# zhangganlin/GlobalSfMpy

Measured on AMD Instinct MI355X. Metric: edge_residuals_per_sec, higher is better.
Workload: dtype f64

## Files before the change

### globalsfmpy_amd/csrc/colsort_kernels.hpp

```cpp
#pragma once
#include "kernels.hpp"

namespace gsfm {

#define GSFM_COL_RB 512
#define GSFM_COL_SUB GSFM_COL_RB
#define GSFM_COL_SLOT_BITS 9
static_assert(GSFM_COL_RB == (1 << GSFM_COL_SLOT_BITS), "row blocks of 512 rows");
#ifndef GSFM_COL_EPL
#define GSFM_COL_EPL 1
#endif
#define GSFM_COL_PAD 0xffffffffu

struct ColWg { uint32_t first_sub, n_sub, row0, part; };
struct ColLayoutDev {
  const ColWg* wg;
  const uint2* meta;
  const uint32_t* kcol;
  const uint16_t* kcnt;
  uint32_t cbits, cmax;
  uint32_t n_wg, nch;
  const uint16_t* k16;
  const uint32_t* kbase;
  const uint32_t* kdel;
};
#define GSFM_K16_CNT_ESC 7u
#define GSFM_K16_DEL_ESC 15u
__host__ __device__ constexpr uint32_t col_pack(uint32_t slot, uint32_t rowcount, uint32_t rowl) { return slot | (rowcount << GSFM_COL_SLOT_BITS) | (rowl << (2 * GSFM_COL_SLOT_BITS + 1)); }
__host__ __device__ __forceinline__ uint32_t col_slot(uint32_t y) { return y & ((1u << GSFM_COL_SLOT_BITS) - 1u); }
__host__ __device__ __forceinline__ uint32_t col_rowcount(uint32_t y) { return (y >> GSFM_COL_SLOT_BITS) & ((2u << GSFM_COL_SLOT_BITS) - 1u); }
__host__ __device__ __forceinline__ uint32_t col_rowl(uint32_t y) { return y >> (2 * GSFM_COL_SLOT_BITS + 1); }
__device__ __forceinline__ uint32_t wave_incl_scan(uint32_t x) {
  int v = (int)x;
  v += __builtin_amdgcn_update_dpp(0, v, 0x111, 0xf, 0xf, false);
  v += __builtin_amdgcn_update_dpp(0, v, 0x112, 0xf, 0xf, false);
  v += __builtin_amdgcn_update_dpp(0, v, 0x114, 0xf, 0xf, false);
  v += __builtin_amdgcn_update_dpp(0, v, 0x118, 0xf, 0xf, false);
  v += __builtin_amdgcn_update_dpp(0, v, 0x142, 0xa, 0xf, false);
  v += __builtin_amdgcn_update_dpp(0, v, 0x143, 0xc, 0xf, false);
  return (uint32_t)v;
}

__device__ __forceinline__ uint2 col_load_meta(const uint2* p) {
  uint2 v;
  v.x = __builtin_nontemporal_load(&p->x); v.y = __builtin_nontemporal_load(&p->y);
  return v;
}

struct ColMatvecArgs {
  ColLayoutDev L;
  const double2 *b0, *b1, *b2;
  const double* u;
  double* part;
  const int* done;
};
template <bool K16, typename Stop>
__device__ __forceinline__ void mv_col_body(const ColMatvecArgs& a, Stop stop_after_request) {
  constexpr int RB = GSFM_COL_RB, EPL = GSFM_COL_EPL;
  __shared__ double slots[2][EPL][3][RB];
  __shared__ uint32_t wtot[2][EPL][RB / 64];
  const ColWg w = a.L.wg[blockIdx.x];
  const uint32_t r = threadIdx.x, wave = r >> 6;
  double y0 = 0.0, y1 = 0.0, y2 = 0.0;
  uint32_t m[EPL], pos[EPL], cbase[EPL]; double2 A[EPL], B[EPL], C[EPL];
  const uint32_t cmask = (1u << a.L.cbits) - 1u, cshift = a.L.cbits + GSFM_COL_SLOT_BITS, cmax = a.L.cmax;
  auto request = [&](uint32_t s) {
#pragma unroll
    for (int k = 0; k < EPL; ++k) {
      const uint32_t sc = w.first_sub + min(s + (uint32_t)k, w.n_sub - 1);
      const size_t e = (size_t)sc * RB + r;
      pos[k] = (uint32_t)e;
      if constexpr (K16) { m[k] = __builtin_nontemporal_load(a.L.k16 + e); cbase[k] = a.L.kbase[(size_t)sc * (RB / 64) + __builtin_amdgcn_readfirstlane(wave)]; }
      else { m[k] = __builtin_nontemporal_load(a.L.kcol + e); cbase[k] = 0u; }
      A[k] = nt_load2(a.b0 + e); B[k] = nt_load2(a.b1 + e); C[k] = nt_load2(a.b2 + e);
    }
  };
  if (w.n_sub) request(0);
  if (stop_after_request()) return;
  int buf = 0;
  for (uint32_t s = 0; s < w.n_sub; s += EPL, buf ^= 1) {
    uint32_t cnt[EPL], inc[EPL];
#pragma unroll
    for (int k = 0; k < EPL; ++k) {
      uint32_t cam, pm, c;
      if constexpr (K16) {
        uint32_t dl = m[k] >> 12;
        if (dl == GSFM_K16_DEL_ESC) dl = a.L.kdel[pos[k]];
        cam = cbase[k] + wave_incl_scan(dl);
        pm = m[k] & ((1u << GSFM_COL_SLOT_BITS) - 1u);
        c = (m[k] >> GSFM_COL_SLOT_BITS) & 7u;
        if (c == GSFM_K16_CNT_ESC) c = a.L.kcnt[pos[k]];
      } else {
        cam = (m[k] & cmask) == cmask ? 0u : (m[k] & cmask); pm = (m[k] >> a.L.cbits) & ((1u << GSFM_COL_SLOT_BITS) - 1u);
        c = m[k] >> cshift;
        if (c == cmax) c = a.L.kcnt[pos[k]];
      }
      const double* um = a.u + 3 * (size_t)cam;
      const double u0 = um[0], u1 = um[1], u2 = um[2];
      slots[buf][k][0][pm] = A[k].x * u0 + A[k].y * u1 + B[k].x * u2;
      slots[buf][k][1][pm] = A[k].y * u0 + B[k].y * u1 + C[k].x * u2;
      slots[buf][k][2][pm] = B[k].x * u0 + C[k].x * u1 + C[k].y * u2;
      cnt[k] = s + (uint32_t)k < w.n_sub ? c : 0u;
      inc[k] = wave_incl_scan(cnt[k]);
      if ((r & 63u) == 63u) wtot[buf][k][wave] = inc[k];
    }
    if (s + EPL < w.n_sub) request(s + EPL);
    __syncthreads();
#pragma unroll
    for (int k = 0; k < EPL; ++k) {
      uint32_t s1 = inc[k];
      for (uint32_t v = 0; v < wave; ++v) s1 += wtot[buf][k][v];
      for (uint32_t t = s1 - cnt[k]; t < s1; ++t) { y0 += slots[buf][k][0][t]; y1 += slots[buf][k][1][t]; y2 += slots[buf][k][2][t]; }
    }
  }
  const size_t o = (size_t)w.part * RB + r, plane = (size_t)a.L.n_wg * RB;
  a.part[o] = y0; a.part[plane + o] = y1; a.part[2 * plane + o] = y2;
}
#define GSFM_K3C_THREADS GSFM_COL_RB
template <bool K16>
__global__ void __launch_bounds__(GSFM_K3C_THREADS) k_mv_col(ColMatvecArgs a) {
  if (a.done && *a.done) return;
  mv_col_body<K16>(a, [] { return false; });
}
struct ColMatvecCgArgs { ColMatvecArgs mv; Cg2Args cg; };
template <bool K16>
__global__ void __launch_bounds__(GSFM_K3C_THREADS) k_mv_col_cg(ColMatvecCgArgs aa) {
  __shared__ double lds[4];
  const Cg2Args& c = aa.cg;
  mv_col_body<K16>(aa.mv, [&]() -> bool {
    const int done = c.sc->done, iters = c.sc->iters;
    const double gamma0 = c.sc->gamma0, tol = c.sc->tol;
    const bool estop = cg_energy_stop(c.sc->einc, c.sc->esum, c.sc->etol2, iters);
    double gpart = 0.0;
    if (threadIdx.x < GSFM_BLOCK) for (int k = threadIdx.x; k < c.nb_cam; k += GSFM_BLOCK) gpart += c.part_g[(size_t)c.par * c.nb_cam + k];
    gpart = wave_sum(gpart);
    if ((threadIdx.x & 63u) == 0 && threadIdx.x < GSFM_BLOCK) lds[threadIdx.x >> 6] = gpart;
    __syncthreads();
    double gamma = 0.0;
#pragma unroll
    for (int k = 0; k < GSFM_BLOCK / 64; ++k) gamma += lds[k];
    if (done) return true;
    bool conv;
    if (c.first) {
      const double rz_abs = c.sc->rz_abs;
      conv = !(gamma > rz_abs);
      if (blockIdx.x == 0 && threadIdx.x == 0) { c.sc->gamma0 = gamma; c.sc->tol = cg_tol_with_floor(tol, rz_abs, gamma); if (conv) { c.sc->done = 1; c.sc->last_rel = 0.0; } }
    } else {
      const double rel = sqrt(gamma / gamma0);
      conv = !(rel > tol) || iters >= c.max_iters || estop;
      if (blockIdx.x == 0 && threadIdx.x == 0) { c.sc->last_rel = rel; if (conv) c.sc->done = 1; }
    }
    return conv;
  });
}
struct ColFinishArgs {
  uint32_t n_rows, row_base, nch, n_wg;
  const double* part; const double* Mblk; const double* p; const double2* q; double* y; const int* done;
  double* dot_part;
};
__global__ void __launch_bounds__(GSFM_BLOCK) k_mv_col_finish(ColFinishArgs a) {
  if (a.done && *a.done) return;
  __shared__ double lds[8];
  const uint32_t row = blockIdx.x * GSFM_BLOCK + threadIdx.x;
  double pAp = 0.0;
  if (row < a.n_rows) {
  const uint32_t blk = row / GSFM_COL_RB, r = row % GSFM_COL_RB;
  const size_t plane = (size_t)a.n_wg * GSFM_COL_RB;
  double t0 = 0.0, t1 = 0.0, t2 = 0.0;
  constexpr uint32_t FB = 8;
  for (uint32_t c0 = 0; c0 < a.nch; c0 += FB) {
    double v0[FB], v1[FB], v2[FB];
#pragma unroll
    for (uint32_t j = 0; j < FB; ++j) {
      const size_t o = ((size_t)blk * a.nch + min(c0 + j, a.nch - 1)) * GSFM_COL_RB + r;
      v0[j] = a.part[o]; v1[j] = a.part[plane + o]; v2[j] = a.part[2 * plane + o];
    }
#pragma unroll
    for (uint32_t j = 0; j < FB; ++j) if (c0 + j < a.nch) { t0 += v0[j]; t1 += v1[j]; t2 += v2[j]; }
  }
  const size_t k = a.row_base + row;
  double R[9], mp[3];
  qmat(load_q(a.q, (uint32_t)k), R);
  sym3_mulvec(a.Mblk + 6 * k, a.p + 3 * k, mp);
  const double y0 = mp[0] - (R[0] * t0 + R[1] * t1 + R[2] * t2), y1 = mp[1] - (R[3] * t0 + R[4] * t1 + R[5] * t2), y2 = mp[2] - (R[6] * t0 + R[7] * t1 + R[8] * t2);
  a.y[3 * k] = y0; a.y[3 * k + 1] = y1; a.y[3 * k + 2] = y2;
  pAp = a.p[3 * k] * y0 + a.p[3 * k + 1] * y1 + a.p[3 * k + 2] * y2;
  }
  if (a.dot_part) {
    const double t = block_sum_bcast(pAp, lds);
    if (threadIdx.x == 0) a.dot_part[blockIdx.x] = t;
  }
}

struct ColRowSArgs {
  ColLayoutDev L;
  uint32_t row_base, n_rows;
  const uint32_t* eid;
  const double2 *qr0, *qr1, *w0, *w1, *w2;
  const double* ws;
  const double2* q;
  double* s_out;
};
template <int F, int WM>
__global__ void __launch_bounds__(GSFM_BLOCK) k_col_s(ColRowSArgs a) {
  constexpr int R = ResDim<F>::R;
  const ColWg w = a.L.wg[blockIdx.x];
  for (uint32_t d = w.first_sub * GSFM_COL_SUB + threadIdx.x; d < (w.first_sub + w.n_sub) * GSFM_COL_SUB; d += GSFM_BLOCK) {
    const uint2 mt = col_load_meta(a.L.meta + d);
    if (mt.x == GSFM_COL_PAD) continue;
    const Quat qk = load_q(a.q, a.row_base + w.row0 + col_rowl(mt.y)), qm = load_q(a.q, mt.x & 0x7fffffffu);
    double2 r0, r1;
    qrel_load<WM>(a.qr0, a.qr1, d, r0, r1);
    const Quat qr = qrel_quat<WM>(r0, r1);
    const EdgeW W = load_w<WM>(a.w0, a.w1, a.w2, a.ws, d);
    double r[R];
    if (mt.x >> 31) edge_residual<F, WM>(qm, qk, qr, W, r);
    else edge_residual<F, WM>(qk, qm, qr, W, r);
    double s = 0.0;
#pragma unroll
    for (int c = 0; c < R; ++c) s += r[c] * r[c];
// ... 229 lines not shown
```

### globalsfmpy_amd/csrc/host_common.hpp

```cpp
#pragma once

#include <dlfcn.h>
#include <hip/hip_runtime.h>

#include <algorithm>
#include <exception>
#include <functional>
#include <stdexcept>
#include <chrono>
#include <cmath>
#include <cstdio>
#include <cstdlib>
#include <cstring>
#include <limits>
#include <sched.h>
#include <string>
#include <thread>
#include <atomic>
#include <vector>

#include "../../include/gsfm_rot.h"
#include "kernels.hpp"
#include "cov_kernels.hpp"
#include "dense_kernels.hpp"
// ... 171 lines not shown
  void destroy() { if (ok) for (int k = 0; k < 2 * NPAIR; ++k) (void)hipEventDestroy(ev[k]); ok = false; }
  int begin(int category) {
    if (!ok || mute || mute_all) return -1;
    if (used == NPAIR) { (void)hipStreamSynchronize(stream); resolve(); }
    const int k = used++;
    cat[k] = category;
    (void)hipEventRecord(ev[2 * k], stream);
    return k;
  }
  void end(int k) { if (k >= 0) (void)hipEventRecord(ev[2 * k + 1], stream); }
  void resolve() {
    for (int k = 0; k < used; ++k) { float ms = 0; if (hipEventElapsedTime(&ms, ev[2 * k], ev[2 * k + 1]) == hipSuccess) acc[cat[k]] += ms; }
    used = 0;
  }
};


}

struct gsfm_rot_problem {
  uint32_t n_cams = 0;
  uint64_t n_edges_in = 0;
  int error_type = 0, functor = F_AA, wmode = W_NONE, param_dim = 3, res_dim = 3;
  bool sharded = false;
  gsfm_rot_shard shard{};
  uint32_t own_begin = 0, own_end = 0, n_rows = 0, n_pad = 0;
  int device = 0;
  hipStream_t stream = nullptr;
  bool own_stream = false;
  struct PcgGraph {
    struct Key {
      int max_iters = 0, stall = 0, chunk = 0; uint32_t coarse = 0; bool lap = false;
      const void* planes = nullptr;
      bool operator==(const Key& k) const { return max_iters == k.max_iters && stall == k.stall && chunk == k.chunk && coarse == k.coarse && lap == k.lap && planes == k.planes; }
    };
    hipGraphExec_t exec = nullptr;
    Key key;
    int collectives = 0;
    bool unusable = false;
    void reset() { if (exec) (void)hipGraphExecDestroy(exec); exec = nullptr; }
  } pcg_graph, pcg2_graph;
  PcgGraph pcg_graph_b, pcg2_graph_b;
  void reset_pcg_graphs() { pcg_graph.reset(); pcg2_graph.reset(); pcg_graph_b.reset(); pcg2_graph_b.reset(); }

  bool q3 = false;
  EdgePlanes cost;
  double cost_n_global = 0.0;
  DevBuf<uint2> cost_idx;
  DevBuf<CostTile> cost_tiles;
  const double2* q_lin = nullptr;
  bool lap = false, lap_capable = false, lin_is_lap = false;
  DevBuf<double> u_rot;
  std::vector<uint32_t> perm;
  std::vector<double> h_cam;
  DevBuf<uint32_t> d_perm;
  int cost_direct = 0;
  EdgePlanes dir;
  DevBuf<uint32_t> row_ptr, col;
  uint32_t G = 16;
  DevBuf<double2> h0, h1, h2, h3;
  DevBuf<double> h4;
  DevBuf<double2> h0_b, h1_b, h2_b;
  DevBuf<double> gD_b;
  int lin_set = 0;
  std::vector<uint32_t> h_cost_eid;

  DevBuf<double> x, x_trial, aa_io, active, scale, gD, Mblk, Minv, Lam, Tinv, b, D6;
// ... 44 lines not shown
  uint64_t loss_epoch = 0;
  hipGraphExec_t dense_graph = nullptr;
  bool dense_graph_lap = false;
  const void* dense_graph_planes = nullptr;
  int nb_mv = 1, mv_reps = 1;
  bool packed = false;
  bool pcg_local = false;
  DevBuf<double> b_own;
  bool component_rest = true;
  uint32_t n_components = 1;
  DevBuf<double> part_a, part_b, part_cost, part_cam, part_gauge, scal;
  DevBuf<CgScalars> cgsc;
  int nb_cam = 1, nb_cost = 1;

  DevLoss h_loss{};
  DevBuf<DevLoss> d_loss;
  DevBuf<double> tables[3];
  gsfm_loss_callback cb = nullptr;
  void* cb_user = nullptr;
  DevBuf<double> rho_ext, s_ext, w_orig;
  std::vector<double> h_s, h_rho;

  struct ColSort {
    bool active = false;
    uint32_t nch = 0, n_wg = 0;
    size_t n_pos = 0;
    DevBuf<ColWg> wg;
    DevBuf<uint2> meta;
    DevBuf<uint32_t> kcol;
    DevBuf<uint16_t> kcnt;
    uint32_t cbits = 0, cmax = 0;
    DevBuf<double> part;
    DevBuf<double> cost_part;
    bool k16_active = false;
    DevBuf<uint16_t> k16;
    DevBuf<uint32_t> kbase, kdel;
    ColLayoutDev dev() const { return ColLayoutDev{wg.p, meta.p, kcol.p, kcnt.p, cbits, cmax, n_wg, nch, k16_active ? k16.p : nullptr, kbase.p, kdel.p}; }
  } cs;

  SigmaDev sigma{};
  bool sigma_pending_cost = false, sigma_pending_lin = false;
  DevBuf<double> sigma_table, sigma_sum;

  bool have_lin = false;
  double* rec_host = nullptr;
  double* rec_dev = nullptr;
  double* mail_host = nullptr;
  double* mail_dev = nullptr;
  DevBuf<double> mail_count;
  double mail_expected = 0.0;
  int mail_state = 0;
  bool loss_staircase = false;
  bool loss_cuts_off = false;
  bool fast_lin_ok = true;
  int graph_launches = 0;
  int n_collectives = 0, n_pcg_collectives = 0, n_pcg_launched = 0;
  std::vector<double> trace;
  EventTimer timer;
};
```

### globalsfmpy_amd/csrc/kernels.hpp

```cpp
#pragma once
#include <hip/hip_runtime.h>
#include <stdint.h>
#include "loss_dev.hpp"
#include "so3_dev.hpp"

namespace gsfm {

enum { F_AA = 0, F_QCOS = 1, F_QNORM = 2, F_RFNORM = 3 };
enum { W_NONE = 0, W_SCALAR = 1, W_MATRIX = 2, W_MATRIX3 = 3  };

template <int F> struct ResDim { static constexpr int R = (F == F_QNORM) ? 4 : (F == F_RFNORM) ? 9 : 3; };

#define GSFM_BLOCK 256
#define GSFM_MAX_PARTIALS 1024
#define GSFM_CAMBLOCK 2048
#ifndef GSFM_TILE_THREADS
#define GSFM_TILE_THREADS 1024
#endif
#ifndef GSFM_K2_ATTR
#define GSFM_K2_ATTR __attribute__((amdgpu_waves_per_eu(3)))
#endif
#ifndef GSFM_GATHER_LOAD
#define GSFM_GATHER_LOAD(p) (*(p))
#endif
// ... 1228 lines not shown
      qt = aa_to_quat(x0, x1, x2);
    } else {
      const size_t k4 = 4 * (size_t)k;
      const Quat q{a.x[k4], a.x[k4 + 1], a.x[k4 + 2], a.x[k4 + 3]};
      const double nd = sqrt(d[0] * d[0] + d[1] * d[1] + d[2] * d[2]);
      qt = q;
      if (nd > 0.0) {
        double sn, cs;
        sincos(nd, &sn, &cs);
        const double kk = sn / nd;
        qt = qmul(Quat{kk * d[0], kk * d[1], kk * d[2], cs}, q);
      }
      a.x_trial[k4] = qt.x; a.x_trial[k4 + 1] = qt.y; a.x_trial[k4 + 2] = qt.z; a.x_trial[k4 + 3] = qt.w;
      const double f0 = q.x - qt.x, f1 = q.y - qt.y, f2 = q.z - qt.z, f3 = q.w - qt.w;
      v[3] = f0 * f0 + f1 * f1 + f2 * f2 + f3 * f3;
      v[4] = act * (qt.x * qt.x + qt.y * qt.y + qt.z * qt.z + qt.w * qt.w);
    }
    a.q_trial[2 * (size_t)k] = make_double2(qt.x, qt.y);
    a.q_trial[2 * (size_t)k + 1] = make_double2(qt.z, qt.w);
  }
#pragma unroll
  for (int c = 0; c < 6; ++c) {
    const double t = block_sum_bcast(v[c], lds);
    if (threadIdx.x == 0) a.partials[(size_t)c * gridDim.x + blockIdx.x] = t;
  }
}
__global__ void __launch_bounds__(GSFM_BLOCK) k_sum_partials_multi(const double* __restrict__ partials, int n, int m, double* out) {
  __shared__ double lds[8];
  for (int c = 0; c < m; ++c) {
    const double t = sum_partials_bcast(partials + (size_t)c * n, n, lds);
    if (threadIdx.x == 0) out[c] = t;
  }
}
__global__ void __launch_bounds__(GSFM_BLOCK) k_cam_norm(const double* __restrict__ x, const double* __restrict__ active,
                                                         uint32_t n, int param_dim, double* partials) {
  __shared__ double lds[8];
  double v = 0.0;
  const uint32_t k = blockIdx.x * GSFM_BLOCK + threadIdx.x;
  if (k < n && active[k] != 0.0) {
    for (int c = 0; c < param_dim; ++c) { const double t = x[(size_t)param_dim * k + c]; v += t * t; }
  }
  const double t = block_sum_bcast(v, lds);
  if (threadIdx.x == 0) partials[blockIdx.x] = t;
}

__global__ void __launch_bounds__(GSFM_BLOCK) k_cam_export(const double* __restrict__ x, const double* __restrict__ gD,
                                                           uint32_t n, int param_dim, double* grad, double* blocks, double* D6) {
  const uint32_t k = blockIdx.x * GSFM_BLOCK + threadIdx.x;
  if (k >= n) return;
  double T[9], Ti[9];
  cam_tangent_maps(x, k, param_dim, T, Ti);
  const double* gd = gD + 9 * (size_t)k;
  const double D[9] = {gd[3], gd[4], gd[5], gd[4], gd[6], gd[7], gd[5], gd[7], gd[8]};
  double DT[9], TDT[9];
  mat3_mul(D, T, DT);
  mat3_tmul(T, DT, TDT);
  for (int c = 0; c < 3; ++c) grad[3 * (size_t)k + c] = T[c] * gd[0] + T[3 + c] * gd[1] + T[6 + c] * gd[2];
  for (int c = 0; c < 9; ++c) blocks[9 * (size_t)k + c] = TDT[c];
  for (int c = 0; c < 6; ++c) D6[6 * (size_t)k + c] = gd[3 + c];
}
__global__ void __launch_bounds__(GSFM_BLOCK) k_cam_apply_T(const double* __restrict__ x, uint32_t n, int param_dim, int transpose,
                                                            const double* __restrict__ in, double* __restrict__ out) {
  const uint32_t k = blockIdx.x * GSFM_BLOCK + threadIdx.x;
  if (k >= n) return;
  double T[9], Ti[9];
  cam_tangent_maps(x, k, param_dim, T, Ti);
// ... 848 lines not shown
```

### globalsfmpy_amd/csrc/problem_create.hpp

```cpp
#pragma once
#include "host_common.hpp"

namespace {

template <typename AdjVec>
bool reorder_for_locality(uint32_t n_cams, uint64_t n_edges, const uint32_t* ei, const uint32_t* ej, const std::vector<uint32_t>& ptr,
                          const AdjVec& adj , std::vector<uint32_t>* perm) {
  perm->clear();
  const char* env = getenv("GSFM_REORDER");
  const int mode = env ? atoi(env) : -1;
  if (mode == 0 || (mode < 0 && n_cams < 2048)) return false;
  double before = 0.0;
  for (uint64_t e = 0; e < n_edges; ++e) before += std::fabs((double)ei[e] - (double)ej[e]);
  before /= (double)n_edges;
  if (mode < 0 && before < 256.0) return false;
  std::vector<uint32_t> stamp(n_cams, 0xffffffffu);
  if (mode < 0) {
    const uint32_t cap = n_cams / 8;
    int flooded = 0;
    for (uint32_t s = 0; s < 32; ++s) {
      const uint32_t c0 = (uint32_t)(((uint64_t)s * n_cams) / 32);
      uint32_t seen = 0;
      for (uint32_t d = ptr[c0]; d < ptr[c0 + 1] && seen < cap; ++d) {
        const uint32_t c1 = adj[d] & 0x7fffffffu;
// ... 142 lines not shown
          const size_t o = base + (e - lo);
          const uint32_t p = (uint32_t)(e - lo), rc = cnt[p + 1] - cnt[p];
          if (e < hi) {
            const uint32_t rl = (uint32_t)(ent[e].first & 0xffff), d = ent[e].second;
            h_col[o] = col[d]; h_eid[o] = deid[d]; h_meta[o] = make_uint2(col[d], col_pack(fill[rl]++, rc, rl));
          } else { h_col[o] = GSFM_COL_PAD; h_eid[o] = 0; h_meta[o] = make_uint2(GSFM_COL_PAD, col_pack(pad_slot++, rc, 0)); }
          h_kcol[o] = (h_meta[o].x == GSFM_COL_PAD ? kpad : (h_meta[o].x & 0x7fffffffu)) | (col_slot(h_meta[o].y) << cbits) | (std::min(rc, cmax) << (cbits + GSFM_COL_SLOT_BITS));
          h_kcnt[o] = (uint16_t)rc;
        }
        if (k16_mode != 0) {
          uint32_t prev = 0, esc = 0;
          for (uint32_t p = 0; p < SUB; ++p) {
            const size_t o = base + p;
            const uint32_t cam = h_meta[o].x == GSFM_COL_PAD ? prev : (h_meta[o].x & 0x7fffffffu);
            uint32_t step = 0;
            if ((p & 63u) == 0) h_kbase[(sub_off[b] + s) * (SUB / 64) + (p >> 6)] = cam; else step = cam - prev;
            prev = cam;
            const uint32_t rc = h_kcnt[o];
            h_kdel[o] = step;
            esc += (step >= GSFM_K16_DEL_ESC) + (rc >= GSFM_K16_CNT_ESC);
            h_k16[o] = (uint16_t)(col_slot(h_meta[o].y) | (std::min(rc, GSFM_K16_CNT_ESC) << GSFM_COL_SLOT_BITS) | (std::min(step, GSFM_K16_DEL_ESC) << 12));
          }
          k16_escapes.fetch_add(esc, std::memory_order_relaxed);
        }
      }
    }
  });
  C.n_wg = (uint32_t)h_wg.size(); C.n_pos = n_pos; C.cbits = cbits; C.cmax = cmax;
  if (k16_mode != 0 && (k16_mode > 0 || (double)k16_escapes.load() <= 0.01 * (double)n_pos)) {
    if (C.k16.upload(h_k16) == hipSuccess && C.kbase.upload(h_kbase) == hipSuccess && C.kdel.upload(h_kdel) == hipSuccess) C.k16_active = true;
    else { (void)hipGetLastError(); C.k16.release(); C.kbase.release(); C.kdel.release(); }
  }
  if (C.wg.upload(h_wg) != hipSuccess || C.meta.upload(h_meta) != hipSuccess || (!C.k16_active && C.kcol.upload(h_kcol) != hipSuccess) || C.kcnt.upload(h_kcnt) != hipSuccess ||
      C.part.alloc((size_t)9 * C.n_wg * RB) != hipSuccess) {
    (void)hipGetLastError();
    C = gsfm_rot_problem::ColSort();
    return 0;
  }
  if (getenv("GSFM_CREATE_TIMING")) fprintf(stderr, "gsfm create: column-sorted layout, %zu positions, 2-byte record %s (%llu escapes)\n", n_pos, C.k16_active ? "on" : "off", (unsigned long long)k16_escapes.load());
  col.swap(h_col); deid.swap(h_eid);
  C.active = true;
  return 0;
}

void run_whiten(gsfm_rot_problem* P, EdgePlanes& pl, const double* d_cov6, const double* d_inl) {
  if (P->wmode == W_NONE || pl.n == 0) return;
  WhitenArgs a{};
  a.cov6 = d_cov6; a.inl = d_inl; a.eid = pl.eid.p; a.n = pl.n; a.error_type = P->error_type;
  a.w0 = pl.w0.p; a.w1 = pl.w1.p; a.w2 = pl.w2.p; a.ws = pl.ws.p;
  hipLaunchKernelGGL(k_whiten, dim3(grid_for(pl.n)), dim3(GSFM_BLOCK), 0, P->stream, a);
}


static gsfm_status problem_create_impl(uint32_t n_cams, uint64_t n_edges, const uint32_t* edge_i_in, const uint32_t* edge_j_in,
                                       const double* rel_aa, int32_t error_type, const double* cov6, const double* inlier_weight,
                                       const gsfm_rot_shard* shard, gsfm_rot_problem** out, gsfm_rot_problem** live) {
  if (!out) return (gsfm_status)fail(GSFM_ERR_INVALID_ARG, "out is NULL");
  *out = nullptr;
  const bool multi_rank = shard && (shard->world_size > 1 || (shard->world_size == 1 && getenv("GSFM_FORCE_SHARD")));
  if (multi_rank && (!shard->all_gather || !shard->all_reduce_sum)) return (gsfm_status)fail(GSFM_ERR_INVALID_ARG, "bad shard descriptor: missing collective callbacks");
  if (const char* why = no_device_reason("the rotation solver")) return (gsfm_status)fail(GSFM_ERR_NO_DEVICE, why);

  gsfm_rot_problem* P = new gsfm_rot_problem;
  *live = P;
  bool agreed = false;
  DevBuf<double> agree_buf;
  double coarse_votes_against = 0.0;
// ... 403 lines not shown
```

### globalsfmpy_amd/csrc/solver_launch.hpp

```cpp
#pragma once
#include "host_common.hpp"

namespace {

int loss_mode(const gsfm_rot_problem* P) {
  if (P->cb) return LM_SIMPLE;
  const DevLoss& L = P->h_loss;
  if (L.n == 0) return LM_SIMPLE;
  if (L.n == 1) {
    const int k = L.nodes[0].kind;
    if (k == GSFM_LOSS_MAGSAC) return (L.nodes[0].nu == 3 && !L.nodes[0].inverse) ? LM_MAGSAC : LM_PROGRAM;
    if (k == GSFM_LOSS_TRIVIAL || k == GSFM_LOSS_HUBER || k == GSFM_LOSS_SOFT_L1 || k == GSFM_LOSS_TUKEY || k == GSFM_LOSS_GEMAN_MCCLURE) return LM_SIMPLE;
  }
  return LM_PROGRAM;
}
template <typename ArgsT, template <int, int, int> class Launcher>
int dispatch(const gsfm_rot_problem* P, const ArgsT& args, int grid) {
  const int f = P->functor, w = (P->wmode == W_MATRIX && P->q3) ? W_MATRIX3 : P->wmode, l = loss_mode(P);
#define GSFM_CASE3(F, W, L) if (f == F && w == W && l == L) { Launcher<F, W, L>::go(args, grid, P->stream); return 0; }
#define GSFM_CASE(F, W) GSFM_CASE3(F, W, LM_PROGRAM) GSFM_CASE3(F, W, LM_SIMPLE) GSFM_CASE3(F, W, LM_MAGSAC)
  GSFM_CASE(F_AA, W_NONE) GSFM_CASE(F_AA, W_SCALAR) GSFM_CASE(F_AA, W_MATRIX) GSFM_CASE(F_AA, W_MATRIX3)
  GSFM_CASE(F_QCOS, W_NONE) GSFM_CASE(F_QNORM, W_NONE) GSFM_CASE(F_RFNORM, W_NONE)
#undef GSFM_CASE
#undef GSFM_CASE3
// ... 248 lines not shown
      CostArgs a = cost_args(P, q);
      a.s_out = P->s_ext.p; a.s_only = 1; a.sigma = P->sigma; a.sigma.on = 1;
      if (dispatch<CostArgs, CostLauncher>(P, a, P->nb_cost)) return fail(GSFM_ERR_UNSUPPORTED, "no kernel for this error type");
      hipLaunchKernelGGL(k_sum_partials, dim3(1), dim3(GSFM_BLOCK), 0, P->stream, P->part_cost.p + P->nb_cost, P->nb_cost, P->sigma_sum.p);
      gsfm_loss_callback keep = P->cb;
      P->cb = nullptr;
      P->sigma_pending_lin = true;
      const int st = launch_lin(P, q);
      P->cb = keep;
      if (st) return st;
    }
    if (int st = refresh_external_rho(P, q)) return st;
  }
  CostArgs a = cost_args(P, q);
  a.rho_ext = P->cb ? P->rho_ext.p : nullptr;
  a.srho_out = out.srho; a.rho12_out = out.rho12; a.rho1_out = out.rho1; a.r_out = out.r; a.s_only = 0;
  if (sig && !P->cb) { a.sigma = P->sigma; a.sigma.on = 1; }
  const int tk = P->timer.begin(T_SWEEP);
  if (dispatch<CostArgs, CostLauncher>(P, a, P->nb_cost)) return fail(GSFM_ERR_UNSUPPORTED, "no kernel for this error type");
  P->timer.end(tk);
  if (reduce) hipLaunchKernelGGL(k_sum_partials, dim3(1), dim3(GSFM_BLOCK), 0, P->stream, P->part_cost.p, P->nb_cost, P->scal.p + slot);
  if (sig && !P->cb) hipLaunchKernelGGL(k_sum_partials, dim3(1), dim3(GSFM_BLOCK), 0, P->stream, P->part_cost.p + P->nb_cost, P->nb_cost, P->sigma_sum.p);
  return all_reduce(P, P->scal.p + slot, 1);
}

bool trial_lin_supported(const gsfm_rot_problem* P) {
  const char* e = getenv("GSFM_TRIAL_LIN");
  if (e && *e && atoi(e) == 0) return false;
  if (!P->h0_b.p || !P->cs.cost_part.p || P->sharded || P->cb || !P->cs.active || !P->lap || P->sigma_pending_cost || P->sigma_pending_lin || !k2_fast_path(P)) return false;
  const int w = (P->wmode == W_MATRIX && P->q3) ? W_MATRIX3 : P->wmode;
  return col_lin_cost_kernel(P->functor, w, loss_mode(P));
}

int launch_lin(gsfm_rot_problem* P, const double2* q, const double* go, bool fused, bool spare) {
  if (fused && !trial_lin_supported(P)) return fail(GSFM_ERR_UNSUPPORTED, "fused trial evaluation without its preconditions");
  if (P->cb) { if (int st = refresh_external_rho(P, q)) return st; }
  LinArgs a{};
  a.n_rows = P->n_rows; a.row_base = P->own_begin; a.G = P->G; a.row_ptr = P->row_ptr.p; a.col = P->col.p; a.eid = P->dir.eid.p;
  a.qr0 = P->dir.qr0.p; a.qr1 = P->dir.qr1.p; a.w0 = P->dir.w0.p; a.w1 = P->dir.w1.p; a.w2 = P->dir.w2.p; a.ws = P->dir.ws.p; a.ws_rw = P->dir.ws.p;
  a.q = q; a.loss = P->d_loss.p; a.rho_ext = P->cb ? P->rho_ext.p : nullptr; a.fast_ok = k2_fast_path(P) ? 1 : 0; a.go = go;
  if (P->sigma_pending_lin) { a.sigma = P->sigma; a.sigma.on = 1; P->sigma_pending_lin = false; }
  if (!P->lap && !P->h3.p && (P->h3.alloc(P->dir.n) != hipSuccess || P->h4.alloc(P->dir.n) != hipSuccess)) return fail(GSFM_ERR_HIP, "allocating the general normal-equation blocks failed");
  a.h0 = P->h0.p; a.h1 = P->h1.p; a.h2 = P->h2.p; a.h3 = P->h3.p; a.h4 = P->h4.p; a.gD = P->gD.p; a.lap = P->lap;
  if (spare) { a.h0 = P->h0_b.p; a.h1 = P->h1_b.p; a.h2 = P->h2_b.p; a.gD = P->gD_b.p; }
  else { P->lin_is_lap = P->lap; P->q_lin = q; }
  const int tk = P->timer.begin(T_LIN);
  if (P->cs.active) {
    ColLinArgs ca{};
    ca.lin = a; ca.L = P->cs.dev(); ca.part = P->cs.part.p; ca.cost_part = fused ? P->cs.cost_part.p : nullptr;
    if (dispatch<ColLinArgs, ColLinLauncher>(P, ca, (int)P->cs.n_wg)) return fail(GSFM_ERR_UNSUPPORTED, "no kernel for this error type");
    const bool body = col_lin_body_frame(P->functor, loss_mode(P) != LM_PROGRAM && !a.rho_ext && a.fast_ok);
    hipLaunchKernelGGL(k_lin_col_finish, dim3(grid_for(P->n_rows)), dim3(GSFM_BLOCK), 0, P->stream, P->n_rows, P->own_begin, P->cs.nch, P->cs.n_wg, (const double*)P->cs.part.p, a.gD,
                       body ? q : (const double2*)nullptr);
  } else if (dispatch<LinArgs, LinLauncher>(P, a, grid_for((size_t)P->n_rows * P->G))) return fail(GSFM_ERR_UNSUPPORTED, "no kernel for this error type");
  P->timer.end(tk);
  if (spare) return 0;
  P->have_lin = true;
  return all_gather(P, P->gD.p, (size_t)P->shard.slice_width * 9);
}

void accept_trial_lin(gsfm_rot_problem* P) {
  std::swap(P->h0.p, P->h0_b.p); std::swap(P->h1.p, P->h1_b.p); std::swap(P->h2.p, P->h2_b.p); std::swap(P->gD.p, P->gD_b.p);
  P->lin_set ^= 1;
  P->lin_is_lap = P->lap; P->q_lin = P->q.p;
  P->have_lin = true;
}

void launch_prep(gsfm_rot_problem* P, const gsfm_rot_options& o, double radius, bool init_scale, const double* radius_dev = nullptr, bool reduce = true) {
  PrepArgs a{};
  a.radius_dev = radius_dev;
  a.n = P->n_cams; a.param_dim = P->param_dim; a.x = P->x.p; a.gD = P->gD.p; a.scale = P->scale.p;
  a.init_scale = init_scale; a.jacobi_scaling = o.jacobi_scaling; a.radius = radius; a.min_diag = o.min_lm_diagonal; a.max_diag = o.max_lm_diagonal;
  a.Mblk = P->Mblk.p; a.Minv = P->Minv.p; a.Lam = P->Lam.p; a.Tinv = P->Tinv.p; a.b = P->b.p; a.gmax_partials = P->part_cam.p;
  hipLaunchKernelGGL(k_cam_prep, dim3(P->nb_cam), dim3(GSFM_BLOCK), 0, P->stream, a);
  if (reduce) {
    hipLaunchKernelGGL(k_max_partials, dim3(1), dim3(GSFM_BLOCK), 0, P->stream, P->part_cam.p, P->nb_cam, P->scal.p + SC_GMAX);
    double* part = P->part_cam.p + (size_t)5 * P->nb_cam;
    hipLaunchKernelGGL(k_cam_bound, dim3(P->nb_cam), dim3(GSFM_BLOCK), 0, P->stream, (const double*)P->Minv.p, (const double*)P->Tinv.p, (const double*)P->active.p, P->n_cams, part);
    hipLaunchKernelGGL(k_max_partials, dim3(1), dim3(GSFM_BLOCK), 0, P->stream, (const double*)part, P->nb_cam, P->scal.p + SC_ZBOUND);
  }
}

int launch_matvec(gsfm_rot_problem* P, const double* Mblk, const double* p, double* y, const int* done, double* dot_part = nullptr, bool* dot_done = nullptr) {
  if (dot_done) *dot_done = false;
  MatvecArgs a{};
  a.n_rows = P->n_rows; a.row_base = P->own_begin; a.G = P->G; a.row_ptr = P->row_ptr.p; a.col = P->col.p;
  a.h0 = P->h0.p; a.h1 = P->h1.p; a.h2 = P->h2.p; a.h3 = P->h3.p; a.h4 = P->h4.p; a.Mblk = Mblk; a.p = p; a.y = y; a.done = done;
  a.q = P->q_lin; a.u = P->u_rot.p;
  if (P->cs.active) {
    auto& c = P->cs;
    ColMatvecArgs m{};
    m.L = c.dev(); m.b0 = P->h0.p; m.b1 = P->h1.p; m.b2 = P->h2.p; m.u = P->u_rot.p; m.part = c.part.p; m.done = done;
    if (c.k16_active) hipLaunchKernelGGL(k_mv_col<true>, dim3(c.n_wg), dim3(GSFM_K3C_THREADS), 0, P->stream, m);
    else hipLaunchKernelGGL(k_mv_col<false>, dim3(c.n_wg), dim3(GSFM_K3C_THREADS), 0, P->stream, m);
    ColFinishArgs f{};
    f.n_rows = P->n_rows; f.row_base = P->own_begin; f.nch = c.nch; f.n_wg = c.n_wg; f.part = c.part.p; f.Mblk = Mblk; f.p = p; f.q = P->q_lin; f.y = y; f.done = done;
    if (dot_part && !P->sharded) { f.dot_part = dot_part; *dot_done = true; }
    hipLaunchKernelGGL(k_mv_col_finish, dim3(grid_for(P->n_rows)), dim3(GSFM_BLOCK), 0, P->stream, f);
    return P->pcg_local ? 0 : all_gather(P, y, (size_t)P->shard.slice_width * 3);
  }
  if (P->lin_is_lap) hipLaunchKernelGGL(k_matvec<true>, dim3(grid_for((size_t)P->n_rows * P->G)), dim3(GSFM_BLOCK), 0, P->stream, a);
  else hipLaunchKernelGGL(k_matvec<false>, dim3(grid_for((size_t)P->n_rows * P->G)), dim3(GSFM_BLOCK), 0, P->stream, a);
  return P->pcg_local ? 0 : all_gather(P, y, (size_t)P->shard.slice_width * 3);
}

}
```

### globalsfmpy_amd/csrc/solver_lm.hpp

```cpp
#pragma once
#include "host_common.hpp"

namespace gsfm {
__global__ void __launch_bounds__(GSFM_BLOCK) k_cam_permute3(const double* __restrict__ src, const uint32_t* __restrict__ perm, uint32_t n, int to_internal, double* __restrict__ dst) {
  const uint32_t k = blockIdx.x * GSFM_BLOCK + threadIdx.x;
  if (k >= n) return;
  const size_t a = to_internal ? k : perm[k], b = to_internal ? perm[k] : k;
  dst[3 * b] = src[3 * a]; dst[3 * b + 1] = src[3 * a + 1]; dst[3 * b + 2] = src[3 * a + 2];
}
}

namespace {

constexpr int GSFM_INTERNAL_RESTART = 1000;

int launch_step(gsfm_rot_problem* P, bool inexact = false, bool reduce = true) {
  StepArgs a{};
  if (inexact && P->lap_capable) {
    const double2* gq = P->q_lin ? P->q_lin : P->q.p;
    GaugeArgs ga{P->n_cams, P->nb_cam, P->active.p, gq, P->Lam.p, P->xcg.p, P->r.p, P->part_gauge.p};
    hipLaunchKernelGGL(k_gauge_part, dim3(P->nb_cam), dim3(GSFM_BLOCK), 0, P->stream, ga);
    a.gauge_part = P->part_gauge.p; a.gauge_nb = P->nb_cam; a.gauge_q = gq;
  }
  a.Minv = inexact ? P->Minv.p : nullptr;
  a.n = P->n_cams; a.param_dim = P->param_dim; a.x = P->x.p; a.active = P->active.p; a.eta = P->xcg.p; a.b = P->b.p; a.rcg = P->r.p;
  a.Lam = P->Lam.p; a.Tinv = P->Tinv.p; a.x_trial = P->x_trial.p; a.q_trial = P->q_trial.p; a.partials = P->part_cam.p;
  hipLaunchKernelGGL(k_cam_step, dim3(P->nb_cam), dim3(GSFM_BLOCK), 0, P->stream, a);
  if (reduce) {
    hipLaunchKernelGGL(k_sum_partials_multi, dim3(1), dim3(GSFM_BLOCK), 0, P->stream, P->part_cam.p, P->nb_cam, 5, P->scal.p + SC_STEP);
    if (inexact) hipLaunchKernelGGL(k_sum_partials, dim3(1), dim3(GSFM_BLOCK), 0, P->stream, P->part_cam.p + (size_t)5 * P->nb_cam, P->nb_cam, P->scal.p + SC_ZL8);
  }
  return 0;
}

int read_scalars(gsfm_rot_problem* P, double* h) {
  static_assert(SC_N <= GSFM_MAIL_WORDS, "the scalar block fits the mailbox");
  if (mail_usable(P)) {
    mail_post(P, P->scal.p, SC_N * sizeof(double));
    P->mail_expected += 1.0;
    return mail_wait(P, h, SC_N * sizeof(double));
  }
  return read_back(P, h, P->scal.p, SC_N * sizeof(double), "read scalars");
}


int evaluate_trial(gsfm_rot_problem* P, bool inexact, double* h, const std::function<bool(const double*)>& fuse_if = nullptr, bool* fused = nullptr) {
  if (fused) *fused = false;
  if (fuse_if && fused && trial_lin_supported(P)) {
    launch_step(P, inexact);
    if (int st = read_scalars(P, h)) return st;
    const bool f = fuse_if(h);
    const double* cpart = P->part_cost.p;
    int ncp = P->nb_cost;
    if (f) {
      if (int st = launch_lin(P, P->q_trial.p, nullptr, true, true)) return st;
      cpart = P->cs.cost_part.p; ncp = (int)P->cs.n_wg;
      *fused = true;
    } else if (int st = launch_cost(P, P->q_trial.p, SC_TRIAL, CostOutputs(), false)) return st;
    if (mail_usable(P)) {
      hipLaunchKernelGGL(k_trial_post, dim3(1), dim3(GSFM_BLOCK), 0, P->stream, P->scal.p, (int)SC_STEP, (int)SC_TRIAL, (const double*)P->part_cam.p, P->nb_cam,
                         cpart, ncp, (int)SC_N, P->mail_dev, P->mail_count.p, inexact ? (int)SC_ZL8 : -1);
// ... 443 lines not shown
    const double n_e = std::fmax(1.0, P->sharded ? P->cost_n_global : (double)P->cost.n);
    const double w = P->loss_staircase ? std::fmin(1.0, 100.0 / std::sqrt(n_e)) : 1e-3, lo = 1.0 / (1.0 + w), hi = 1.0 + w;
    return r.cc > 0.0 && ((r.sn > lo * pt && r.sn <= hi * pt) || (acc > lo * ft && acc <= hi * ft) || (r.rd > lo * o.min_relative_decrease && r.rd <= hi * o.min_relative_decrease));
  }
  void reject() { radius /= decrease_factor; decrease_factor *= 2.0; sum->num_unsuccessful_steps++; prev_accepted = false; }
  int accept(const Step& s, const Row& row, double cand_cost) {
    std::swap(P->x.p, P->x_trial.p);
    HIPCHK(hipMemcpyAsync(P->q.p, P->q_trial.p, 32 * (size_t)P->n_cams, hipMemcpyDeviceToDevice, P->stream));
    x_norm = std::sqrt(h[SC_STEP + 4]);
    x_cost = cand_cost;
    if (trial_fused) accept_trial_lin(P);
    else if (int st = launch_lin(P, P->q.p)) return st;
    sum->num_residual_sweeps++; sum->num_linearizations++;
    prev_accepted = true;
    radius = radius / std::fmax(1.0 / 3.0, 1.0 - std::pow(2.0 * row.rd - 1.0, 3));
    radius = std::fmin(o.max_trust_region_radius, radius);
    decrease_factor = 2.0;
    launch_prep(P, o, radius, false);
    prep_valid = true;
    if (defer_gmax) {
      HIPCHK(hipMemcpyAsync((void*)gmax_pin, P->scal.p + SC_GMAX, sizeof(double), hipMemcpyDeviceToHost, P->stream));
      gmax_deferred = true;
      gmax_trace_slot = P->trace.size() + 3;
    } else {
      if (int st = read_scalars(P, h)) return st;
      gmax = h[SC_GMAX];
    }
    if (s.step_loose) loose_applied = true;
    return count_accepted(row);
  }
};

int lm_solve(gsfm_rot_problem* P, const gsfm_rot_options& o_in, gsfm_rot_summary* sum) {
  LmSolve lm{P, o_in, o_in, sum};
  if (int r = lm.start(); r != LM_GO_ON) return r;
  while (true) {
    LmSolve::Step s;
    int r = lm.begin_iteration(s);
    if (r == LM_GO_ON && s.exact_now && lm.device_control && !lm.exact_pipeline_broken) r = lm.exact_device_iteration();
    if (r == LM_GO_ON) r = lm.component_step(s);
    if (r == LM_GO_ON) r = lm.pcg_step(s);
    if (r == LM_GO_ON) r = lm.decide(s);
    if (r != LM_NEXT) return r;
  }
}

}
```

### globalsfmpy_amd/csrc/solver_pcg.hpp

```cpp
#pragma once
#include "host_common.hpp"

namespace {

bool spd_inverse(std::vector<double>& A, size_t n, std::vector<double>& inv) {
  for (size_t j = 0; j < n; ++j) {
    double d = A[j * n + j];
    for (size_t k = 0; k < j; ++k) d -= A[j * n + k] * A[j * n + k];
    if (!(d > 0.0) || !std::isfinite(d)) return false;
    const double l = std::sqrt(d);
    A[j * n + j] = l;
    for (size_t i = j + 1; i < n; ++i) {
      double v = A[i * n + j];
      for (size_t k = 0; k < j; ++k) v -= A[i * n + k] * A[j * n + k];
      A[i * n + j] = v / l;
    }
  }
  std::vector<double> Li(n * n, 0.0);
  for (size_t i = 0; i < n; ++i) {
    double* ri = &Li[i * n];
    ri[i] = 1.0;
    for (size_t k = 0; k < i; ++k) {
      const double l = A[i * n + k];
      const double* rk = &Li[k * n];
// ... 88 lines not shown
}

struct PcgStagnation {
  double mark_rel = 1.0; int mark_it = 0;
  bool stop(int iters, double rel) {
    if (rel < 0.5 * mark_rel) { mark_rel = rel; mark_it = iters; return false; }
    return iters >= 1000 && iters - mark_it >= 512;
  }
};

double pcg_abs_floor2(const gsfm_rot_problem* P) { const double f = (P->n_components > 1 && !P->loss_staircase && !P->cb && P->component_rest) ? 1e-11 : 2e-14; return f * f; }
double comp_freeze_below(const gsfm_rot_problem* P) { return (!P->loss_staircase && !P->cb && P->component_rest) ? 1e-10 : 0.0; }

struct PcgLoop {
  gsfm_rot_problem::PcgGraph& G;
  bool blocked;
  bool& unusable;
  int key_stall; uint32_t key_coarse;
  bool clamp_chunks; int cap_slack;
};

template <class Scalars, class Iter>
int pcg_chunk_loop(gsfm_rot_problem* P, const gsfm_rot_options& o, const PcgLoop& L, Scalars* sc, Iter&& enqueue_iter, double tol, double etol2,
                   int launched, int* iters_out, double* rel_out) {
  const int chunk = std::max(1, o.cg_check_interval);
  const bool mail = mail_usable(P);
  auto enqueue_chunk = [&]() -> int {
    for (int c = 0; c < chunk; ++c) if (int st = enqueue_iter()) return st;
    if (mail) mail_post(P, sc, sizeof(Scalars));
    return 0;
  };
  auto& G = L.G;
  bool graph = o.pcg_hip_graph && (!P->sharded || P->pcg_local || graph_collectives_ok(P, o)) && chunk % 2 == 0 && !L.blocked;
  const gsfm_rot_problem::PcgGraph::Key key{o.max_cg_iterations, L.key_stall, chunk, L.key_coarse, P->lin_is_lap, P->h0.p};
  if (graph && (!G.exec || !(G.key == key))) {
    G.reset();
    hipGraph_t captured = nullptr;
    if (hipStreamBeginCapture(P->stream, hipStreamCaptureModeThreadLocal) == hipSuccess) {
      const int c0 = P->n_collectives, p0 = P->n_pcg_collectives;
      const int st = enqueue_chunk();
      const hipError_t e = hipStreamEndCapture(P->stream, &captured);
      G.collectives = P->n_collectives - c0;
      P->n_collectives = c0; P->n_pcg_collectives = p0;
      if (st == 0 && e == hipSuccess && captured && hipGraphInstantiate(&G.exec, captured, nullptr, nullptr, 0) == hipSuccess) G.key = key;
      else G.exec = nullptr;
      if (captured) (void)hipGraphDestroy(captured);
    }
    if (!G.exec) { (void)hipGetLastError(); L.unusable = true; graph = false; }
  }
  int chunks = 1; PcgStagnation stagnation; Scalars h{};
  while (true) {
    const int tk = P->timer.begin(T_CG);
    for (int c = 0; c < chunks; ++c) {
      if (graph) { HIPCHK(hipGraphLaunch(G.exec, P->stream)); P->graph_launches++; P->n_collectives += G.collectives; P->n_pcg_collectives += G.collectives; }
      else if (int st = enqueue_chunk()) return st;
      launched += chunk; P->n_pcg_launched += chunk;
      if (mail) P->mail_expected += 1.0;
    }
    P->timer.end(tk);
    if (int st = mail ? mail_wait(P, &h, sizeof(h)) : read_back(P, &h, sc, sizeof(h), "pcg")) return st;
    if (h.done || launched >= o.max_cg_iterations + chunk + L.cap_slack || stagnation.stop(h.iters, h.last_rel)) break;
    chunks = 1;
    if (!(etol2 > 0.0) && h.iters > 0 && h.last_rel > 0.0 && h.last_rel < 1.0 && tol > 0.0 && tol < h.last_rel) {
      const double per_iter = std::log(h.last_rel) / h.iters;
      const double remaining = std::log(tol / h.last_rel) / per_iter;
      chunks = (int)std::min(8.0, std::max(1.0, std::ceil(remaining / chunk)));
    }
// ... 141 lines not shown
```

Before: 8.593 billion.

## Fuse column matvec finish into matvec via last-block-done counters

```diff
diff --git a/globalsfmpy_amd/csrc/colsort_kernels.hpp b/globalsfmpy_amd/csrc/colsort_kernels.hpp
--- a/globalsfmpy_amd/csrc/colsort_kernels.hpp
+++ b/globalsfmpy_amd/csrc/colsort_kernels.hpp
@@ -54,8 +54,39 @@
   double* part;
   const int* done;
 };
-template <bool K16, typename Stop>
-__device__ __forceinline__ void mv_col_body(const ColMatvecArgs& a, Stop stop_after_request) {
+struct ColFinishArgs {
+  uint32_t n_rows, row_base, nch, n_wg;
+  const double* part; const double* Mblk; const double* p; const double2* q; double* y; const int* done;
+  double* dot_part;
+};
+__device__ __forceinline__ double mv_col_finish_row(const ColFinishArgs& a, uint32_t row) {
+  const uint32_t blk = row / GSFM_COL_RB, r = row % GSFM_COL_RB;
+  const size_t plane = (size_t)a.n_wg * GSFM_COL_RB;
+  double t0 = 0.0, t1 = 0.0, t2 = 0.0;
+  constexpr uint32_t FB = 8;
+  for (uint32_t c0 = 0; c0 < a.nch; c0 += FB) {
+    double v0[FB], v1[FB], v2[FB];
+#pragma unroll
+    for (uint32_t j = 0; j < FB; ++j) {
+      const size_t o = ((size_t)blk * a.nch + min(c0 + j, a.nch - 1)) * GSFM_COL_RB + r;
+      v0[j] = a.part[o]; v1[j] = a.part[plane + o]; v2[j] = a.part[2 * plane + o];
+    }
+#pragma unroll
+    for (uint32_t j = 0; j < FB; ++j) if (c0 + j < a.nch) { t0 += v0[j]; t1 += v1[j]; t2 += v2[j]; }
+  }
+  const size_t k = a.row_base + row;
+  double R[9], mp[3];
+  qmat(load_q(a.q, (uint32_t)k), R);
+  sym3_mulvec(a.Mblk + 6 * k, a.p + 3 * k, mp);
+  const double y0 = mp[0] - (R[0] * t0 + R[1] * t1 + R[2] * t2), y1 = mp[1] - (R[3] * t0 + R[4] * t1 + R[5] * t2), y2 = mp[2] - (R[6] * t0 + R[7] * t1 + R[8] * t2);
+  a.y[3 * k] = y0; a.y[3 * k + 1] = y1; a.y[3 * k + 2] = y2;
+  return a.p[3 * k] * y0 + a.p[3 * k + 1] * y1 + a.p[3 * k + 2] * y2;
+}
+#ifndef GSFM_K3C_PUB_WT
+#define GSFM_K3C_PUB_WT 1
+#endif
+template <bool K16, typename Stop, bool FIN = false>
+__device__ __forceinline__ void mv_col_body(const ColMatvecArgs& a, Stop stop_after_request, const ColFinishArgs* f = nullptr, uint32_t* fin_cnt = nullptr) {
   constexpr int RB = GSFM_COL_RB, EPL = GSFM_COL_EPL;
   __shared__ double slots[2][EPL][3][RB];
   __shared__ uint32_t wtot[2][EPL][RB / 64];
@@ -114,13 +145,52 @@
     }
   }
   const size_t o = (size_t)w.part * RB + r, plane = (size_t)a.L.n_wg * RB;
-  a.part[o] = y0; a.part[plane + o] = y1; a.part[2 * plane + o] = y2;
+  if (FIN && GSFM_K3C_PUB_WT) {
+    __hip_atomic_store(a.part + o, y0, __ATOMIC_RELAXED, __HIP_MEMORY_SCOPE_AGENT);
+    __hip_atomic_store(a.part + plane + o, y1, __ATOMIC_RELAXED, __HIP_MEMORY_SCOPE_AGENT);
+    __hip_atomic_store(a.part + 2 * plane + o, y2, __ATOMIC_RELAXED, __HIP_MEMORY_SCOPE_AGENT);
+  } else {
+    a.part[o] = y0; a.part[plane + o] = y1; a.part[2 * plane + o] = y2;
+  }
+  if constexpr (FIN) {
+    asm volatile("s_waitcnt vmcnt(0)" ::: "memory");
+    __syncthreads();
+    uint32_t* last = &wtot[0][0][0];
+    if (r == 0) {
+      if (!GSFM_K3C_PUB_WT) { __builtin_amdgcn_fence(__ATOMIC_RELEASE, "agent"); asm volatile("s_waitcnt vmcnt(0)" ::: "memory"); }
+      const uint32_t b = w.row0 / RB;
+      const uint32_t t = __hip_atomic_fetch_add(fin_cnt + b, 1u, __ATOMIC_RELAXED, __HIP_MEMORY_SCOPE_AGENT);
+      *last = t == f->nch - 1;
+      if (t == f->nch - 1) {
+        __hip_atomic_store(fin_cnt + b, 0u, __ATOMIC_RELAXED, __HIP_MEMORY_SCOPE_AGENT);
+        __builtin_amdgcn_fence(__ATOMIC_ACQUIRE, "agent");
+        asm volatile("s_waitcnt vmcnt(0)" ::: "memory");
+      }
+    }
+    __syncthreads();
+    if (!*last) return;
+    const uint32_t row = w.row0 + r;
+    const double pAp = row < f->n_rows ? mv_col_finish_row(*f, row) : 0.0;
+    if (f->dot_part) {
+      double* lds = &slots[0][0][0][0];
+      const double v = wave_sum(pAp);
+      if ((r & 63u) == 0) lds[wave] = v;
+      __syncthreads();
+      if ((r & (GSFM_BLOCK - 1)) == 0) {
+        double t = 0;
+        for (int k = 0; k < GSFM_BLOCK / 64; ++k) t += lds[(r / 64) + k];
+        const uint32_t ob = row / GSFM_BLOCK;
+        if (ob * GSFM_BLOCK < f->n_rows) f->dot_part[ob] = t;
+      }
+    }
+  }
 }
 #define GSFM_K3C_THREADS GSFM_COL_RB
-template <bool K16>
-__global__ void __launch_bounds__(GSFM_K3C_THREADS) k_mv_col(ColMatvecArgs a) {
+template <bool K16, bool FIN = false>
+__global__ void __launch_bounds__(GSFM_K3C_THREADS) k_mv_col(ColMatvecArgs a, ColFinishArgs f, uint32_t* cnt) {
   if (a.done && *a.done) return;
-  mv_col_body<K16>(a, [] { return false; });
+  auto no_stop = [] { return false; };
+  mv_col_body<K16, decltype(no_stop), FIN>(a, no_stop, &f, cnt);
 }
 struct ColMatvecCgArgs { ColMatvecArgs mv; Cg2Args cg; };
 template <bool K16>
@@ -153,39 +223,11 @@
     return conv;
   });
 }
-struct ColFinishArgs {
-  uint32_t n_rows, row_base, nch, n_wg;
-  const double* part; const double* Mblk; const double* p; const double2* q; double* y; const int* done;
-  double* dot_part;
-};
 __global__ void __launch_bounds__(GSFM_BLOCK) k_mv_col_finish(ColFinishArgs a) {
   if (a.done && *a.done) return;
   __shared__ double lds[8];
   const uint32_t row = blockIdx.x * GSFM_BLOCK + threadIdx.x;
-  double pAp = 0.0;
-  if (row < a.n_rows) {
-  const uint32_t blk = row / GSFM_COL_RB, r = row % GSFM_COL_RB;
-  const size_t plane = (size_t)a.n_wg * GSFM_COL_RB;
-  double t0 = 0.0, t1 = 0.0, t2 = 0.0;
-  constexpr uint32_t FB = 8;
-  for (uint32_t c0 = 0; c0 < a.nch; c0 += FB) {
-    double v0[FB], v1[FB], v2[FB];
-#pragma unroll
-    for (uint32_t j = 0; j < FB; ++j) {
-      const size_t o = ((size_t)blk * a.nch + min(c0 + j, a.nch - 1)) * GSFM_COL_RB + r;
-      v0[j] = a.part[o]; v1[j] = a.part[plane + o]; v2[j] = a.part[2 * plane + o];
-    }
-#pragma unroll
-    for (uint32_t j = 0; j < FB; ++j) if (c0 + j < a.nch) { t0 += v0[j]; t1 += v1[j]; t2 += v2[j]; }
-  }
-  const size_t k = a.row_base + row;
-  double R[9], mp[3];
-  qmat(load_q(a.q, (uint32_t)k), R);
-  sym3_mulvec(a.Mblk + 6 * k, a.p + 3 * k, mp);
-  const double y0 = mp[0] - (R[0] * t0 + R[1] * t1 + R[2] * t2), y1 = mp[1] - (R[3] * t0 + R[4] * t1 + R[5] * t2), y2 = mp[2] - (R[6] * t0 + R[7] * t1 + R[8] * t2);
-  a.y[3 * k] = y0; a.y[3 * k + 1] = y1; a.y[3 * k + 2] = y2;
-  pAp = a.p[3 * k] * y0 + a.p[3 * k + 1] * y1 + a.p[3 * k + 2] * y2;
-  }
+  const double pAp = row < a.n_rows ? mv_col_finish_row(a, row) : 0.0;
   if (a.dot_part) {
     const double t = block_sum_bcast(pAp, lds);
     if (threadIdx.x == 0) a.dot_part[blockIdx.x] = t;
diff --git a/globalsfmpy_amd/csrc/host_common.hpp b/globalsfmpy_amd/csrc/host_common.hpp
--- a/globalsfmpy_amd/csrc/host_common.hpp
+++ b/globalsfmpy_amd/csrc/host_common.hpp
@@ -227,7 +227,8 @@
     struct Key {
       int max_iters = 0, stall = 0, chunk = 0; uint32_t coarse = 0; bool lap = false;
       const void* planes = nullptr;
-      bool operator==(const Key& k) const { return max_iters == k.max_iters && stall == k.stall && chunk == k.chunk && coarse == k.coarse && lap == k.lap && planes == k.planes; }
+      bool fused = false;
+      bool operator==(const Key& k) const { return max_iters == k.max_iters && stall == k.stall && chunk == k.chunk && coarse == k.coarse && lap == k.lap && planes == k.planes && fused == k.fused; }
     };
     hipGraphExec_t exec = nullptr;
     Key key;
@@ -338,6 +339,7 @@
     uint32_t cbits = 0, cmax = 0;
     DevBuf<double> part;
     DevBuf<double> cost_part;
+    DevBuf<uint32_t> fin_cnt;
     bool k16_active = false;
     DevBuf<uint16_t> k16;
     DevBuf<uint32_t> kbase, kdel;
@@ -349,6 +351,7 @@
   DevBuf<double> sigma_table, sigma_sum;
 
   bool have_lin = false;
+  bool fused_chain = true;
   double* rec_host = nullptr;
   double* rec_dev = nullptr;
   double* mail_host = nullptr;
diff --git a/globalsfmpy_amd/csrc/kernels.hpp b/globalsfmpy_amd/csrc/kernels.hpp
--- a/globalsfmpy_amd/csrc/kernels.hpp
+++ b/globalsfmpy_amd/csrc/kernels.hpp
@@ -1284,6 +1284,13 @@
     if (threadIdx.x == 0) out[c] = t;
   }
 }
+__global__ void __launch_bounds__(GSFM_BLOCK) k_sum_partials_multi_plus(const double* __restrict__ partials, int n, int m, double* out, double* out_extra) {
+  __shared__ double lds[8];
+  for (int c = 0; c <= m; ++c) {
+    const double t = sum_partials_bcast(partials + (size_t)c * n, n, lds);
+    if (threadIdx.x == 0) *(c < m ? out + c : out_extra) = t;
+  }
+}
 __global__ void __launch_bounds__(GSFM_BLOCK) k_cam_norm(const double* __restrict__ x, const double* __restrict__ active,
                                                          uint32_t n, int param_dim, double* partials) {
   __shared__ double lds[8];
diff --git a/globalsfmpy_amd/csrc/problem_create.hpp b/globalsfmpy_amd/csrc/problem_create.hpp
--- a/globalsfmpy_amd/csrc/problem_create.hpp
+++ b/globalsfmpy_amd/csrc/problem_create.hpp
@@ -198,7 +198,7 @@
     else { (void)hipGetLastError(); C.k16.release(); C.kbase.release(); C.kdel.release(); }
   }
   if (C.wg.upload(h_wg) != hipSuccess || C.meta.upload(h_meta) != hipSuccess || (!C.k16_active && C.kcol.upload(h_kcol) != hipSuccess) || C.kcnt.upload(h_kcnt) != hipSuccess ||
-      C.part.alloc((size_t)9 * C.n_wg * RB) != hipSuccess) {
+      C.part.alloc((size_t)9 * C.n_wg * RB) != hipSuccess || C.fin_cnt.alloc(C.n_wg / C.nch, true) != hipSuccess) {
     (void)hipGetLastError();
     C = gsfm_rot_problem::ColSort();
     return 0;
diff --git a/globalsfmpy_amd/csrc/solver_launch.hpp b/globalsfmpy_amd/csrc/solver_launch.hpp
--- a/globalsfmpy_amd/csrc/solver_launch.hpp
+++ b/globalsfmpy_amd/csrc/solver_launch.hpp
@@ -304,6 +304,11 @@
   return col_lin_cost_kernel(P->functor, w, loss_mode(P));
 }
 
+bool fused_chain_enabled() {
+  const char* e = getenv("GSFM_FUSED_CHAIN");
+  return !(e && *e && atoi(e) == 0);
+}
+
 int launch_lin(gsfm_rot_problem* P, const double2* q, const double* go, bool fused, bool spare) {
   if (fused && !trial_lin_supported(P)) return fail(GSFM_ERR_UNSUPPORTED, "fused trial evaluation without its preconditions");
   if (P->cb) { if (int st = refresh_external_rho(P, q)) return st; }
@@ -363,11 +368,17 @@
     auto& c = P->cs;
     ColMatvecArgs m{};
     m.L = c.dev(); m.b0 = P->h0.p; m.b1 = P->h1.p; m.b2 = P->h2.p; m.u = P->u_rot.p; m.part = c.part.p; m.done = done;
-    if (c.k16_active) hipLaunchKernelGGL(k_mv_col<true>, dim3(c.n_wg), dim3(GSFM_K3C_THREADS), 0, P->stream, m);
-    else hipLaunchKernelGGL(k_mv_col<false>, dim3(c.n_wg), dim3(GSFM_K3C_THREADS), 0, P->stream, m);
     ColFinishArgs f{};
     f.n_rows = P->n_rows; f.row_base = P->own_begin; f.nch = c.nch; f.n_wg = c.n_wg; f.part = c.part.p; f.Mblk = Mblk; f.p = p; f.q = P->q_lin; f.y = y; f.done = done;
     if (dot_part && !P->sharded) { f.dot_part = dot_part; *dot_done = true; }
+    const bool fin = P->fused_chain && f.dot_part && c.fin_cnt.p;
+    if (fin) {
+      if (c.k16_active) hipLaunchKernelGGL((k_mv_col<true, true>), dim3(c.n_wg), dim3(GSFM_K3C_THREADS), 0, P->stream, m, f, c.fin_cnt.p);
+      else hipLaunchKernelGGL((k_mv_col<false, true>), dim3(c.n_wg), dim3(GSFM_K3C_THREADS), 0, P->stream, m, f, c.fin_cnt.p);
+      return P->pcg_local ? 0 : all_gather(P, y, (size_t)P->shard.slice_width * 3);
+    }
+    if (c.k16_active) hipLaunchKernelGGL(k_mv_col<true>, dim3(c.n_wg), dim3(GSFM_K3C_THREADS), 0, P->stream, m, ColFinishArgs{}, (uint32_t*)nullptr);
+    else hipLaunchKernelGGL(k_mv_col<false>, dim3(c.n_wg), dim3(GSFM_K3C_THREADS), 0, P->stream, m, ColFinishArgs{}, (uint32_t*)nullptr);
     hipLaunchKernelGGL(k_mv_col_finish, dim3(grid_for(P->n_rows)), dim3(GSFM_BLOCK), 0, P->stream, f);
     return P->pcg_local ? 0 : all_gather(P, y, (size_t)P->shard.slice_width * 3);
   }
diff --git a/globalsfmpy_amd/csrc/solver_lm.hpp b/globalsfmpy_amd/csrc/solver_lm.hpp
--- a/globalsfmpy_amd/csrc/solver_lm.hpp
+++ b/globalsfmpy_amd/csrc/solver_lm.hpp
@@ -26,7 +26,8 @@
   a.n = P->n_cams; a.param_dim = P->param_dim; a.x = P->x.p; a.active = P->active.p; a.eta = P->xcg.p; a.b = P->b.p; a.rcg = P->r.p;
   a.Lam = P->Lam.p; a.Tinv = P->Tinv.p; a.x_trial = P->x_trial.p; a.q_trial = P->q_trial.p; a.partials = P->part_cam.p;
   hipLaunchKernelGGL(k_cam_step, dim3(P->nb_cam), dim3(GSFM_BLOCK), 0, P->stream, a);
-  if (reduce) {
+  if (reduce && inexact && P->fused_chain) hipLaunchKernelGGL(k_sum_partials_multi_plus, dim3(1), dim3(GSFM_BLOCK), 0, P->stream, P->part_cam.p, P->nb_cam, 5, P->scal.p + SC_STEP, P->scal.p + SC_ZL8);
+  else if (reduce) {
     hipLaunchKernelGGL(k_sum_partials_multi, dim3(1), dim3(GSFM_BLOCK), 0, P->stream, P->part_cam.p, P->nb_cam, 5, P->scal.p + SC_STEP);
     if (inexact) hipLaunchKernelGGL(k_sum_partials, dim3(1), dim3(GSFM_BLOCK), 0, P->stream, P->part_cam.p + (size_t)5 * P->nb_cam, P->nb_cam, P->scal.p + SC_ZL8);
   }
@@ -536,6 +537,7 @@
 };
 
 int lm_solve(gsfm_rot_problem* P, const gsfm_rot_options& o_in, gsfm_rot_summary* sum) {
+  P->fused_chain = fused_chain_enabled();
   LmSolve lm{P, o_in, o_in, sum};
   if (int r = lm.start(); r != LM_GO_ON) return r;
   while (true) {
diff --git a/globalsfmpy_amd/csrc/solver_pcg.hpp b/globalsfmpy_amd/csrc/solver_pcg.hpp
--- a/globalsfmpy_amd/csrc/solver_pcg.hpp
+++ b/globalsfmpy_amd/csrc/solver_pcg.hpp
@@ -144,7 +144,7 @@
   };
   auto& G = L.G;
   bool graph = o.pcg_hip_graph && (!P->sharded || P->pcg_local || graph_collectives_ok(P, o)) && chunk % 2 == 0 && !L.blocked;
-  const gsfm_rot_problem::PcgGraph::Key key{o.max_cg_iterations, L.key_stall, chunk, L.key_coarse, P->lin_is_lap, P->h0.p};
+  const gsfm_rot_problem::PcgGraph::Key key{o.max_cg_iterations, L.key_stall, chunk, L.key_coarse, P->lin_is_lap, P->h0.p, P->fused_chain};
   if (graph && (!G.exec || !(G.key == key))) {
     G.reset();
     hipGraph_t captured = nullptr;
```

Measured after the change: 8.652 billion (median of 5 runs). Within noise of the previous version (+0.7%).
